# Jonetz/TreeDetection

Hardware: AMD Instinct MI355X
Metric: tiles/sec (1000x1000 RGB+nDSM) predict_tiles model stage (higher is better)
Workload: dtype f32

## Files before the change

treedetection_amd/csrc/api.cpp:

```cpp
#include "common.h"
#include "detect.h"
#include <cstdarg>
#include <cstdio>
#include <cmath>
#include <cstdlib>
#include <cstring>
#include <vector>


namespace {
td_status scratch(void** p, size_t bytes) {
    TD_HIP_CHECK(hipMalloc(p, bytes ? bytes : 16));
    return TD_OK;
}
}

extern "C" {

void td_model_desc_default(td_model_desc* d) {
    d->num_classes = 1;
    d->precision = TD_PRECISION_FP32;
    d->pre_nms_topk = 1000;
    d->post_nms_topk = 1000;
    d->detections_per_image = 100;
// ... 136 lines not shown
    const char* tenv = getenv("TD_WINO_TILE");
    const bool f43 = head_w || (tenv && atoi(tenv) == 4);
    const int P = f43 ? 36 : 16;
    const size_t T = f43 ? (size_t)B * ((H + 3) / 4) * ((W + 3) / 4) : (size_t)B * ((H + 1) / 2) * ((W + 1) / 2);
    std::vector<float> wh((size_t)Cout * 9 * Cin), uh((size_t)P * Cout * Cin);
    TD_HIP_CHECK(hipMemcpy(wh.data(), w, wh.size() * sizeof(float), hipMemcpyDeviceToHost));
    if (f43) wino43_filter_transform(wh.data(), Cout, Cin, uh.data());
    else wino_filter_transform(wh.data(), Cout, Cin, uh.data());
    void *U = nullptr, *V = nullptr, *Mb = nullptr;
    td_status st;
    if ((st = scratch(&U, uh.size() * 4)) < 0 || (st = scratch(&V, P * T * Cin * 4)) < 0 || (st = scratch(&Mb, P * T * Cout * 4)) < 0) {
        (void)hipFree(U); (void)hipFree(V); (void)hipFree(Mb);
        return st;
    }
    TD_HIP_CHECK(hipMemcpy(U, uh.data(), uh.size() * 4, hipMemcpyHostToDevice));
    const char* folde = getenv("TD_WINO_FOLD");
    const bool fold = f43 && !head_w && folde && atoi(folde) != 0;
    if (fold) TD_REQUIRE(wino43_fused_ok(B, H, W, Cin, Cout), "td_conv2d_winograd_nhwc: TD_WINO_FOLD needs Cin %% 128 == 0, Cout %% 64 == 0");
    const char* fenv = getenv("TD_WINO_FUSED");
    WinoRun r{};
    r.form = fold ? CONV_WINO43_FOLD : f43 ? CONV_WINO43 : CONV_WINO22;
    r.fused_input = !fenv || atoi(fenv) != 0;
    r.slab_tiles = (int)T; r.fold_group = B;
    r.x = x; r.U = static_cast<float*>(U); r.scale = scale; r.bias = bias; r.y = y;
    r.B = B; r.H = H; r.W = W; r.cin = Cin; r.cout = Cout; r.relu = relu;
    r.V = static_cast<float*>(V); r.M = static_cast<float*>(Mb); r.m_mul = 1; r.gemm_cfg = -1;
    r.head_w = head_w; r.head_b = head_b; r.head_y = head_y; r.head_n = head_n;
    st = wino_run(r, s);
    hipError_t herr = hipStreamSynchronize(s);
    (void)hipFree(U); (void)hipFree(V); (void)hipFree(Mb);
    if (st < 0) return st;
    TD_HIP_CHECK(herr);
    return TD_OK;
}

td_status td_resize_tile_u8(const uint8_t* src, int h, int w, int c, uint8_t* dst, int out_h, int out_w,
                            int dst_pitch_px, void* tmp_dev, void* stream) {
    return resize_tile_u8_launch(src, h, w, c, dst, out_h, out_w, dst_pitch_px, tmp_dev, static_cast<hipStream_t>(stream));
}

td_status td_resize_batch_u8(const uint8_t* const* src_tiles, int n, int h, int w, int c, uint8_t* dst, int out_h,
                             int out_w, int dst_pitch_px, int64_t dst_image_stride_bytes, void* tmp_dev, void* stream) {
    return resize_batch_u8_launch(src_tiles, n, h, w, c, dst, out_h, out_w, dst_pitch_px, (size_t)dst_image_stride_bytes,
                                  tmp_dev, static_cast<hipStream_t>(stream));
}
// ... 161 lines not shown
```

treedetection_amd/csrc/common.h:

```cpp
#pragma once
#include <hip/hip_runtime.h>
#include <hip/hip_fp16.h>
#include <cstdint>
#include <cstddef>
#include "../../include/treedet.h"
#include "conv_path.h"
#include <string>
#include <vector>

void td_set_error(const char* fmt, ...);

int td_polygons_json_text(const int32_t* mask_region, const int64_t* mask_offset, const uint32_t* mask_bits, int64_t mask_words,
                          const float* scores, const int32_t* classes, int n, const double* transform, const char* image_id,
                          std::string& out, const char* who);

#define TD_HIP_CHECK(expr)                                                                         \
    do {                                                                                           \
        hipError_t _e = (expr);                                                                    \
        if (_e != hipSuccess) {                                                                    \
            td_set_error("%s failed: %s (%s:%d)", #expr, hipGetErrorString(_e), __FILE__, __LINE__); \
            return TD_ERR_HIP;                                                                     \
        }                                                                                          \
    } while (0)

// ... 99 lines not shown
    {TILE_SPLIT,   1, TILE_F32, false, false, 22, 0,   0,  0},
    {TILE_SPLIT,   2, TILE_F32, false, false, 23, 0,   0,  0},
    {TILE_SPLIT,   3, TILE_F32, false, false, 24, 0,   0,  0},
};
static inline const ConvTile* conv_tile(int id) { return id >= 0 && id < (int)(sizeof TD_CONV_TILES / sizeof *TD_CONV_TILES) ? &TD_CONV_TILES[id] : nullptr; }
static inline bool conv_head_capable(int id, int precision) { return precision == TD_PRECISION_FP16 && conv_tile(id) && conv_tile(id)->head; }
const char* conv_tile_refusal(int id, const ConvArgs& a, int precision);
td_status conv2d_launch(const ConvArgs& a, int precision, hipStream_t stream);
td_status conv_pp8_grouped_launch(ConvArgs a, hipStream_t stream);
void conv_bd_pack(const void* w_ohwi, int elem_bytes, int cout, int kh, int kw, int cin, std::vector<unsigned char>& out);
bool conv_bd_ok(const ConvArgs& a, int precision);
td_status conv_bd_launch(const ConvArgs& a, int precision, int variant, hipStream_t stream);
bool conv_bs_ok(const ConvArgs& a, int precision);
td_status conv_bs_launch(const ConvArgs& a, int precision, hipStream_t stream);
void conv_split_pack(const float* w, int cout, int cin, std::vector<unsigned char>& out, int taps = 1);
bool conv_split_ok(const ConvArgs& a, int precision);
td_status conv_split_launch(const ConvArgs& a, int variant, hipStream_t stream);
td_status wino_gemm_launch(const ConvArgs& a, hipStream_t stream);

struct TailArgs {
    const void* x;
    const void* w2;
    const float* scale2;
    const float* bias2;
    const void* w3;
    const float* scale3;
    const float* bias3;
    const void* res;
    void* y;
    int B, H, W, MID, COUT, M;
// ... 11 lines not shown
void wino_filter_transform(const float* w_ohwi, int N, int C, float* U);
td_status wino43_input_launch(const float* x, int B, int H, int W, int C, float* V, const int* m_dyn, hipStream_t s);
td_status wino43_fused_launch(const float* V, const float* U, int B, int H, int W, int C, int N, const float* scale, const float* bias,
                              int relu, float* y, const int* m_dyn, hipStream_t s);
td_status wino43_output_launch(const float* Mb, int B, int H, int W, int N, const float* scale, const float* bias, int relu,
                               float* y, const int* m_dyn, hipStream_t s);
td_status wino43_output_head_launch(const float* Mb, int B, int H, int W, int N, const float* scale, const float* bias, int relu,
                                    const float* head_w, const float* head_b, float* head_y, int head_n, hipStream_t s);
void wino43_filter_transform(const float* w_ohwi, int N, int C, float* U);
struct WinoRun {
    int form;
    bool fused_input;
    int slab_tiles;
    int fold_group;
    const float *x, *U, *scale, *bias;
    float* y;
    int B, H, W, cin, cout, relu;
    float *V, *M;
    const int* m_dyn;
    int m_mul;
    int gemm_cfg;
    const float *head_w, *head_b;
    float* head_y;
    int head_n;
};
ConvArgs wino_plane_args(const WinoRun& r, int n, long long t0);
ConvArgs wino43_plane_args(const WinoRun& r);
enum { WINO_STEP_INPUT, WINO_STEP_GEMM, WINO_STEP_OUTPUT };
struct WinoHook {
    void* ctx;
// ... 26 lines not shown
```

treedetection_amd/csrc/conv_igemm.hip:

```cpp
#include "common.h"
#include <cstdlib>
#include <type_traits>

#include "conv_tiles.h"

namespace {

template <typename T, typename TO, int MT, int NT, int NSTAGE, int WM, int WN>
__global__ __launch_bounds__(64 * WM * WN, NSTAGE == 1 && MT * NT <= 4 ? 4 : 1)
void conv_igemm_kernel(const ConvArgs a_in) {
    ConvArgs a = a_in;
    if (a.batch_count > 1) {
        const long long bz = blockIdx.y;
        a.x = static_cast<const T*>(a.x) + bz * a.x_bs;
        a.w = static_cast<const T*>(a.w) + bz * a.w_bs;
        a.y = static_cast<TO*>(a.y) + bz * a.y_bs;
    }
    constexpr int THREADS = 64 * WM * WN;
    constexpr int BM = 32 * MT * WM, BN = 32 * NT * WN;
    constexpr int LDROWS = THREADS / 8;
    constexpr int AROWS = BM / LDROWS, BROWS = BN / LDROWS;
    static_assert(BM % LDROWS == 0 && BN % LDROWS == 0 && LDROWS % 16 == 0, "tile / thread-count mismatch");
    constexpr int ES = sizeof(T);
    constexpr int KE = Elem<T>::PER_CHUNK;
// ... 913 lines not shown
    const ConvTile* t = conv_tile(id);
    if (!t) return id < 0 ? nullptr : "no such tile id";
    if (t->family == TILE_RETIRED)
        return "a retired experiment (stream-K / the 4-wave 256x256 tile) that lost to the block tiles and left the library";
    const unsigned prec_bit = precision == TD_PRECISION_FP16 ? TILE_F16 : precision == TD_PRECISION_FP32 ? TILE_F32 : 0;
    if (!(t->prec & prec_bit)) return t->prec == TILE_F16 ? "fp16-only tile" : "fp32-only tile";
    if (t->family == TILE_PP8 && (a.out_mode != 0 || a.batch_count > 1)) return "plain output, no batched launch only";
    if (t->family == TILE_PLANE && !(a.KH == 1 && a.KW == 1 && a.stride == 1 && a.pad == 0 && a.out_mode == 0 && a.res_shift == 0 && !a.out_f32 &&
                                     a.m_off == 0 && a.Cin >= 32 && a.Cin % 32 == 0 && a.M > 0 && a.Cout > 0 && (a.batch_count <= 1 || !a.res) &&
                                     (size_t)a.M * a.Cin * 4 < 0xfffffff0ull - (1u << 20)))
        return "plane-only tile (fp32 1x1, stride 1, no padding, no upsampled residual, Cin a multiple of 32)";
    if (t->family == TILE_BS && !conv_bs_ok(a, precision))
        return "conv_bs_ok failed (1x1, stride 1, 1 / 2 / 4 k-chunks, 128 <= Cout <= 2048, Cout % 8 == 0, packed filters)";
    if (t->family == TILE_BD && !conv_bd_ok(a, precision)) return "conv_bd_ok failed (packed filters, plain output)";
    if (t->family == TILE_SPLIT && !conv_split_ok(a, precision))
        return "conv_split_ok failed (fp32 1x1 without padding, plain output, Cin a multiple of 32, split filter bank)";
    return nullptr;
}

td_status conv2d_launch(const ConvArgs& a, int precision, hipStream_t stream) {
    TD_REQUIRE(precision == TD_PRECISION_FP32 || precision == TD_PRECISION_FP16, "conv2d: bad precision %d", precision);
    int cfg = a.tile_cfg;
    if (cfg < 0) {
        const char* forced = getenv("TD_CONV_CFG");
        if (forced) cfg = atoi(forced);
    }
    if (const char* why = conv_tile_refusal(cfg, a, precision)) {
        if (a.tile_strict || !conv_tile(cfg) || conv_tile(cfg)->family == TILE_RETIRED) {
            td_set_error("conv2d: tile_cfg %d cannot run this launch%s: %s", cfg, a.tile_strict ? " (strict tile selection)" : "", why);
            return TD_ERR_INVALID;
        }
        cfg = -1;
    }
    const int ke = precision == TD_PRECISION_FP16 ? 64 : 32;
    TD_REQUIRE(a.Cin % ke == 0, "conv2d: Cin=%d must be a multiple of %d", a.Cin, ke);
    TD_REQUIRE(a.M > 0 && a.Cout > 0, "conv2d: empty problem (M=%d, Cout=%d)", a.M, a.Cout);
    const size_t es = precision == TD_PRECISION_FP16 ? 2 : 4;
    TD_REQUIRE((size_t)a.B * a.H * a.W * (size_t)a.Cin * es < 0xfffffff0ull - (1u << 20), "conv2d: input tensor must stay below 4 GB (32-bit buffer offsets)");
    TD_REQUIRE((size_t)a.Cout * a.KH * a.KW * a.Cin * es < 0xfffffff0ull - (1u << 20), "conv2d: weight tensor must stay below 4 GB");
    TD_REQUIRE(a.KH * a.KW <= 32, "conv2d: at most 32 filter taps (got %dx%d)", a.KH, a.KW);
    TD_REQUIRE(a.out_mode == 0 || (a.Cout % 32 == 0 && !a.res), "conv2d: bad deconv configuration");
    TD_REQUIRE(!a.head_w || (conv_head_capable(cfg, precision) && a.Cout == 256 && !a.res && a.out_mode == 0 && a.head_y && a.head_n >= 1 && a.head_n <= 32),
               "conv2d: a fused head needs a 256-channel fp16 layer on a tile that owns all its channels (tile id %d)", cfg);
    if (cfg < 0) {
        const bool small_m = a.M <= 64 * 256;
        cfg = a.Cout <= 64 ? (small_m ? 3 : 1) : (small_m ? 2 : 0);
    }
    const ConvTile& t = *conv_tile(cfg);
    if (t.family == TILE_BS) return conv_bs_launch(a, precision, stream);
    if (t.family == TILE_BD) return conv_bd_launch(a, precision, t.variant, stream);
    if (t.family == TILE_SPLIT) return conv_split_launch(a, t.variant, stream);
    TD_REQUIRE(a.batch_count <= 1 || (a.KH == 1 && a.KW == 1 && !a.res), "conv2d: batched launches are 1x1 contractions");
    if (t.family == TILE_PP8) return a.out_f32 ? pp8_launch<float>(a, stream) : pp8_launch<_Float16>(a, stream);
    if (t.family == TILE_PLANE) return plane_launch(a, cfg, stream);
    if (precision == TD_PRECISION_FP32) return dispatch<float, float>(a, cfg, stream);
    if (a.out_f32) return dispatch<_Float16, float>(a, cfg, stream);
    return dispatch<_Float16, _Float16>(a, cfg, stream);
}
// ... 1 lines not shown
```

treedetection_amd/csrc/conv_path.cpp:

```cpp
#include "conv_path.h"
#include "../../include/treedet.h"

#include <algorithm>

bool wino43_fused_ok(int B, int H, int W, int C, int N) {
    const long long T = (long long)B * ((H + 3) / 4) * ((W + 3) / 4);
    return (C == 128 || C == 256 || C == 512) && N >= 64 && N % 64 == 0 && 36ull * (unsigned long long)T * C * 4 < 0xfffffff0ull - (1u << 20) &&
           36ull * (unsigned long long)N * C * 4 < 0xfffffff0ull - (1u << 20) && (unsigned long long)B * H * W * N * 4 < 0xfffffff0ull - (1u << 20);
}

ConvPath conv_path(const ConvRules& r, const ConvSite& s) {
    const ConvLayerFacts& L = s.L;
    const int Ho = (s.H + 2 * s.pad - L.kh) / s.stride + 1, Wo = (s.W + 2 * s.pad - L.kw) / s.stride + 1;
    const bool fp32 = r.precision == TD_PRECISION_FP32;
    const int maxc = std::max(L.cin, L.cout);
    ConvPath p{};
    p.head = HEAD_OWN_LAUNCH;
    p.slab_tiles = r.wino_slab > 0 ? r.wino_slab : (1 << 30);
    auto key = [&](int k2, long long rows, int flags) {
        p.tune = true;
        p.key[0] = L.cout; p.key[1] = L.cin; p.key[2] = k2; p.key[3] = (int)rows; p.key[4] = flags;
    };
    const bool head1x1 = s.has_head && r.fuse_head && !s.m_dyn && s.relu && L.cout == 256 && s.head.cin == 256 && s.head.kh == 1 && s.head.kw == 1 &&
                         s.head.cout <= 32 && !s.head.scale;
// ... 19 lines not shown
    }
    const int hw = s.H * s.W, wf = r.wino_fold;
    const bool head = s.has_head, dyn = s.m_dyn;
    const bool fold = wf > 0 && wino43_fused_ok(dyn ? s.B : 1, s.H, s.W, L.cin, L.cout) &&
                      (((wf & 1) && !dyn && (!head || (wf & 32)) && ((L.cin == 256 && hw >= 160 * 160) || (L.cin == 128 && hw >= 80 * 80))) ||
                       ((wf & 2) && dyn && !head) || ((wf & 4) && !dyn && !head && L.cin == 256 && hw >= 80 * 80) ||
                       ((wf & 8) && !dyn && !head && hw >= 40 * 40) || ((wf & 16) && !dyn && !head));
    if (fold) {
        p.form = CONV_WINO43_FOLD;
        const unsigned long long room = 0xfffffff0ull - (2u << 20);
        const unsigned long long gmax = std::min(room / (36ull * tiles_img * (unsigned long long)maxc * 4ull), room / (16ull * tiles_img * L.cout * 4ull));
        p.fold_group = dyn ? s.B : (int)std::max<unsigned long long>(1ull, std::min<unsigned long long>(gmax, s.B));
        return p;
    }
    p.form = CONV_WINO43;
    key(1 * 16 + 1, T43, 4 + 64);
    if (head1x1) p.head = HEAD_IN_TRANSFORM;
    return p;
}
```

treedetection_amd/csrc/conv_path.h:

```cpp
#pragma once
#include <cstddef>

struct ConvRules {
    int precision;
    bool winograd;
    bool wino_fused;
    int wino_minc;
    int wino43_min;
    int wino_fold;
    int wino_slab;
    bool fuse_head;
    size_t wino_elems;
};
struct ConvLayerFacts {
    int cout, cin, kh, kw;
    bool scale, out_f32;
    bool wino_u, wino_u43, w_split;
};
struct ConvSite {
    ConvLayerFacts L;
    int B, H, W, stride, pad;
    bool relu, res;
    int out_mode;
    bool m_dyn;
    int m_mul;
    bool has_head;
    ConvLayerFacts head;
};

enum ConvForm { CONV_DIRECT, CONV_SPLIT, CONV_WINO22, CONV_WINO43, CONV_WINO43_FOLD };
enum ConvHead { HEAD_OWN_LAUNCH, HEAD_IN_TRANSFORM, HEAD_IF_TILE_OWNS_256 };

struct ConvPath {
    ConvForm form;
    ConvHead head;
    bool tune;
    int key[5];
    int slab_tiles;
    int fold_group;
};

ConvPath conv_path(const ConvRules& r, const ConvSite& s);

bool wino43_fused_ok(int B, int H, int W, int C, int N);
```

treedetection_amd/csrc/conv_split.hip:

```cpp
#include "common.h"
#include "conv_tiles.h"
#include <utility>

namespace {

typedef unsigned u32x4 __attribute__((ext_vector_type(4)));

template <int... R, class F>
__device__ __forceinline__ void static_for(std::integer_sequence<int, R...>, F&& f) {
    (f(std::integral_constant<int, R>{}), ...);
}

template <int MT, int NT, int WM, int WN>
__device__ __forceinline__ void conv_split_body(const ConvArgs& a, char* lds) {
    constexpr int THREADS = 64 * WM * WN;
    constexpr int BM = 32 * MT * WM, BN = 32 * NT * WN;
    constexpr int LDROWS = THREADS / 8;
    constexpr int AROWS = BM / LDROWS;
    static_assert(BM % LDROWS == 0 && AROWS >= 1 && LDROWS % 16 == 0, "tile / thread-count mismatch");
    char* As = lds;

    int M = a.M;
    if (a.m_dyn) {
        int md = *a.m_dyn * a.m_mul - a.m_off;
// ... 188 lines not shown
            step(std::integral_constant<int, 1>{}, std::integral_constant<int, 1>{}, it + 1);
        }
        if (it + 2 < nit) {
            step(std::integral_constant<int, 2>{}, std::integral_constant<int, 0>{}, it + 2);
            step(std::integral_constant<int, 2>{}, std::integral_constant<int, 1>{}, it + 2);
        }
    }
    asm volatile("s_waitcnt vmcnt(0)" ::: "memory");
    asm volatile("s_waitcnt lgkmcnt(0)" ::: "memory");
    __builtin_amdgcn_s_barrier();
    conv_epilogue<float, float, MT, NT, WM, WN, 1>(a, acc, lds, M, m0, n0, tid, lane, wm, wn);
}

template <int MT, int NT, int WM, int WN, int WPE>
__global__ __launch_bounds__(64 * WM * WN, WPE)
void conv_split_kernel(const ConvArgs a) {
    constexpr int STAGE_BYTES = 3 * 32 * MT * WM * CHUNK_BYTES;
    constexpr int EPI_BYTES = conv_epilogue_lds_bytes<float, MT, NT, WM, WN, 1>();
    constexpr int LDS_BYTES = STAGE_BYTES > EPI_BYTES ? STAGE_BYTES : EPI_BYTES;
    constexpr int BLOCKS_PER_CU = 4 * WPE / (WM * WN) > 0 ? 4 * WPE / (WM * WN) : 1;
    static_assert(LDS_BYTES * BLOCKS_PER_CU <= 160 * 1024, "the blocks the registers allow on a CU must fit its LDS");
    __shared__ __attribute__((aligned(16))) char lds[LDS_BYTES];
    conv_split_body<MT, NT, WM, WN>(a, lds);
}

template <int MT, int NT, int WM, int WN, int WPE>
td_status launch_split(const ConvArgs& a, hipStream_t stream) {
    const int tiles = td_cdiv(a.M, 32 * MT * WM) * td_cdiv(a.Cout, 32 * NT * WN);
    hipLaunchKernelGGL((conv_split_kernel<MT, NT, WM, WN, WPE>), dim3(tiles), dim3(64 * WM * WN), 0, stream, a);
    TD_KERNEL_CHECK();
    return TD_OK;
}

inline unsigned short bf16_rne(float f) {
    unsigned u = __builtin_bit_cast(unsigned, f);
    if ((u & 0x7fffffffu) > 0x7f800000u) return (unsigned short)((u >> 16) | 0x40);
    u += 0x7fffu + ((u >> 16) & 1u);
    return (unsigned short)(u >> 16);
}

}

void conv_split_pack(const float* w, int cout, int cin, std::vector<unsigned char>& out, int taps) {
    const int nit = taps * (cin / 32), nt32 = (cout + 31) / 32;
// ... 5 lines not shown
                for (int l = 0; l < 64; ++l) {
                    const int n = t * 32 + (l & 31), h = l >> 5;
                    if (n >= cout) continue;
                    const int cc = c / taps, tap = c - cc * taps;
                    for (int e = 0; e < 8; ++e) {
                        float v = w[((size_t)n * taps + tap) * cin + (size_t)cc * 32 + 16 * s + 8 * (e >> 2) + 4 * h + (e & 3)];
                        for (int p = 0; p < 3; ++p) {
                            const unsigned short b = bf16_rne(v);
                            o[(((((size_t)t * nit + c) * 2 + s) * 3 + p) * 64 + l) * 8 + e] = b;
                            v = v - __builtin_bit_cast(float, (unsigned)b << 16);
                        }
                    }
                }
}

bool conv_split_ok(const ConvArgs& a, int precision) {
    return precision == TD_PRECISION_FP32 && a.w_split && a.KH == 1 && a.KW == 1 && a.pad == 0 && a.stride >= 1 && a.out_mode == 0 &&
           a.batch_count <= 1 && !a.out_f32 && !a.head_w && a.Cin >= 32 && a.Cin % 32 == 0 &&
           (size_t)((a.Cout + 31) / 32) * (size_t)(a.Cin / 32) * SPLIT_CHUNK_BYTES < 0xfffffff0ull - (1u << 20);
}

td_status conv_split_launch(const ConvArgs& a, int variant, hipStream_t stream) {
    TD_REQUIRE(conv_split_ok(a, TD_PRECISION_FP32), "split-bf16 contraction: unsupported launch (fp32 1x1 without padding, split filter bank)");
    switch (variant) {
        case 3: return launch_split<2, 2, 1, 2, 2>(a, stream);
        case 2: return launch_split<2, 4, 1, 2, 1>(a, stream);
        case 1: return launch_split<2, 2, 2, 2, 2>(a, stream);
        default: return launch_split<4, 2, 1, 4, 1>(a, stream);
    }
}
```

treedetection_amd/csrc/engine.cpp:

```cpp
#include "common.h"
#include "detect.h"
#include "workspace.h"

#include <cmath>
#include <cstdio>
#include <cstdlib>
#include <cstring>
#include <algorithm>
#include <functional>
#include <map>
#include <optional>
#include <string>
#include <tuple>
#include <vector>

namespace {

struct HostTensor {
    const float* data = nullptr;
    std::vector<int64_t> shape;
    int64_t numel() const {
        int64_t n = 1;
        for (auto s : shape) n *= s;
        return n;
    }
};

enum { SPLIT_FC = 1, SPLIT_LATERAL = 2, SPLIT_CONV1 = 4, SPLIT_CONV3 = 8, SPLIT_SHORTCUT = 16,
       SPLIT_DEFAULT = SPLIT_FC | SPLIT_LATERAL | SPLIT_CONV1 | SPLIT_SHORTCUT };

struct ConvLayer {
    int cout = 0, cin = 0, kh = 1, kw = 1;
    void* w = nullptr;
    float* scale = nullptr;
    float* bias = nullptr;
    bool out_f32 = false;
    void* w_frag = nullptr;
    void* w_split = nullptr;
    void* w_tail_split = nullptr;
    float* wino_u = nullptr;
    float* wino_u43 = nullptr;
};

struct Block {
    ConvLayer c1, c2, c3, sc;
    bool has_sc = false;
    int stride = 1;
};

struct NamedTensor { void* p; WsDims dims; int elem; };

}

struct td_engine : Workspace {
    td_model_desc desc{};
    int device = 0;
// ... 22 lines not shown
    int backbone_subbatch = 0;
    std::map<std::tuple<int, int, int, int, int>, int> tuned;
    bool winograd = true;
    size_t wino_elems = 0;
    bool group_levels = true;
    bool fuse_head = true;
    bool fuse_tail = true;
    bool fuse_tail_fp16 = false;
    bool wino_fused = true;
    int wino_slab = 0;
    int wino_minc = 128;
    int wino43_min = 12;
    int wino_fold = 39;
    int f32_split = SPLIT_DEFAULT;
    bool f32_split_tail = true;
    std::string tune_cache;
    void* tune_evict = nullptr;
    size_t tune_evict_bytes = 0;

    struct FwdCtx {
        const void* images = nullptr;
        int input_format = 0, B = 0, Hp = 0, Wp = 0;
        ImgSizes valid{}, outsz{};
        td_detections out{};
        bool valid_ctx = false;
    } ctx;
    hipEvent_t phase_ev[7] = {};
    bool phase_ev_recorded[7] = {};
    hipEvent_t prev5_ev = nullptr;
    bool prev5_recorded = false;
// ... 136 lines not shown
        td_set_error("load_weights: norm tensors of '%s' do not have %d channels", p.c_str(), c);
        return TD_ERR_WEIGHTS;
    }
    scale.resize(c);
    bias.resize(c);
    for (int i = 0; i < c; ++i) {
        const float r = 1.0f / std::sqrt(v->data[i] + 1e-5f);
        const float s = g->data[i] * r;
        const float ms = m->data[i] * s;
        scale[i] = s;
        bias[i] = b->data[i] - ms;
    }
    return TD_OK;
}

td_status upload_wino(td_engine* e, const std::vector<float>& w_ohwi, ConvLayer& L) {
    L.wino_u = nullptr;
    if (e->desc.precision != TD_PRECISION_FP32 || !e->winograd || L.kh != 3 || L.kw != 3 || L.cin % 32 != 0 || L.cout % 4 != 0)
        return TD_OK;
    std::vector<float> u((size_t)16 * L.cout * L.cin);
    wino_filter_transform(w_ohwi.data(), L.cout, L.cin, u.data());
    td_status st = upload(e, u, &L.wino_u);
    if (st < 0 || e->wino43_min <= 0 || L.cin < e->wino_minc || L.cout < e->wino_minc) return st;
    std::vector<float> u43((size_t)36 * L.cout * L.cin);
    wino43_filter_transform(w_ohwi.data(), L.cout, L.cin, u43.data());
    return upload(e, u43, &L.wino_u43);
}

td_status load_conv_bn(td_engine* e, const TensorMap& tm, const std::string& p, ConvLayer& L, int split_cls = 0) {
    const HostTensor* w;
    td_status st = need(tm, p + ".weight", 4, &w);
    if (st < 0) return st;
    L.cout = (int)w->shape[0];
    L.cin = (int)w->shape[1];
    L.kh = (int)w->shape[2];
    L.kw = (int)w->shape[3];
    const std::vector<float> packed = pack_ohwi(*w);
    if ((st = upload_w(e, packed, &L.w)) < 0) return st;
    if ((st = upload_frag(e, packed, L)) < 0) return st;
    if ((st = upload_split(e, packed, L, split_cls)) < 0) return st;
    if ((st = upload_wino(e, packed, L)) < 0) return st;
    std::vector<float> s, b;
    if ((st = bn_fold(tm, p, L.cout, s, b)) < 0) return st;
    if ((st = upload(e, s, &L.scale)) < 0) return st;
    return upload(e, b, &L.bias);
}

td_status load_conv_bias(td_engine* e, const TensorMap& tm, const std::string& p, ConvLayer& L, int split_cls = 0) {
    const HostTensor *w, *b;
    td_status st = need(tm, p + ".weight", 4, &w);
    if (st < 0) return st;
    if ((st = need(tm, p + ".bias", 1, &b)) < 0) return st;
    L.cout = (int)w->shape[0];
    L.cin = (int)w->shape[1];
    L.kh = (int)w->shape[2];
    L.kw = (int)w->shape[3];
    if (b->shape[0] != L.cout) {
        td_set_error("load_weights: bias of '%s' has wrong length", p.c_str());
        return TD_ERR_WEIGHTS;
    }
    const std::vector<float> packed = pack_ohwi(*w);
    if ((st = upload_w(e, packed, &L.w)) < 0) return st;
    if ((st = upload_frag(e, packed, L)) < 0) return st;
    if ((st = upload_split(e, packed, L, split_cls)) < 0) return st;
    if ((st = upload_wino(e, packed, L)) < 0) return st;
    L.scale = nullptr;
    return upload(e, std::vector<float>(b->data, b->data + L.cout), &L.bias);
}

WsGeom engine_geom(const td_engine* e, int B, int Hp, int Wp) {
    int32_t c[WS_WIDTHS] = {e->stem_c};
    for (int s = 0; s < 4; ++s) { c[1 + s] = e->stages[s][0].c1.cout; c[5 + s] = e->stages[s][0].c2.cout; c[9 + s] = e->stages[s][0].c3.cout; }
    c[13] = e->fpn_c; c[14] = e->fc_dim; c[15] = e->deconv.cout / 4;
    return ws_geom(e->desc.precision, e->winograd, e->desc.post_nms_topk, e->desc.detections_per_image, c, B, Hp, Wp);
}

void publish(td_engine* e, const WsGeom& g, int phase) {
    for (const WsRow& r : ws_rows())
        for (int i = 0; r.pub && (r.phase == phase || (phase == 0 && r.phase == TD_PHASE_STEM)) && i < r.count; ++i) {
            char name[32];
// ... 107 lines not shown
    TD_REQUIRE(d.precision == TD_PRECISION_FP32 || d.precision == TD_PRECISION_FP16, "td_engine_create: bad precision %d", d.precision);
    TD_REQUIRE(d.pre_nms_topk >= 1 && d.pre_nms_topk <= RPN_CAND, "td_engine_create: pre_nms_topk must be in [1,%d]", RPN_CAND);
    TD_REQUIRE(d.post_nms_topk >= 1 && d.post_nms_topk <= 1024, "td_engine_create: post_nms_topk must be in [1,1024]");
    TD_REQUIRE(d.detections_per_image >= 1 && d.detections_per_image <= 1024, "td_engine_create: detections_per_image must be in [1,1024]");
    int ndev = 0;
    TD_HIP_CHECK(hipGetDeviceCount(&ndev));
    TD_REQUIRE(device >= 0 && device < ndev, "td_engine_create: device %d of %d", device, ndev);
    TD_HIP_CHECK(hipSetDevice(device));
    td_engine* e = new td_engine();
    if (const char* sbenv = getenv("TD_BACKBONE_SUBBATCH")) e->backbone_subbatch = atoi(sbenv);
    if (const char* tc = getenv("TD_TUNE_CACHE")) e->tune_cache = tc;
    if (const char* gl = getenv("TD_GROUP_LEVELS")) e->group_levels = atoi(gl) != 0;
    if (const char* ft = getenv("TD_FUSE_TAIL")) { e->fuse_tail = atoi(ft) != 0; e->fuse_tail_fp16 = atoi(ft) == 2; }
    if (const char* sp = getenv("TD_F32_SPLIT")) e->f32_split = atoi(sp);
    if (const char* spt = getenv("TD_F32_SPLIT_TAIL")) e->f32_split_tail = atoi(spt) != 0;
    e->desc = d;
    read_rule_switches(e);
    load_tune_cache(e);
    e->device = device;
    *out = e;
    return TD_OK;
}

void td_engine_destroy(td_engine* e) {
    if (!e) return;
    (void)hipSetDevice(e->device);
    free_pool(e->weight_allocs);
    free_pool(e->ws_allocs);
    if (e->tune_evict) (void)hipFree(e->tune_evict);
    for (auto& r : e->prof_recs) { (void)hipEventDestroy(r.a); (void)hipEventDestroy(r.b); }
// ... 68 lines not shown
            std::vector<unsigned short> w16;
            std::vector<float> b16;
            stem_mfma_prepare(p.data(), s.data(), b.data(), e->stem_c, w16, b16);
            if ((st = upload(e, w16, &e->stem_w16)) < 0) return st;
            if ((st = upload(e, b16, &e->stem_bias16)) < 0) return st;
        }
    }
    for (int si = 0; si < 4; ++si) {
        e->stages[si].clear();
        for (int bi = 0;; ++bi) {
            const std::string p = "backbone.bottom_up.res" + std::to_string(si + 2) + "." + std::to_string(bi);
            if (tm.find(p + ".conv1.weight") == tm.end()) break;
            Block blk;
            blk.stride = (bi == 0 && si > 0) ? 2 : 1;
            if ((st = load_conv_bn(e, tm, p + ".conv1", blk.c1, si > 0 ? SPLIT_CONV1 : 0)) < 0) return st;
            if ((st = load_conv_bn(e, tm, p + ".conv2", blk.c2)) < 0) return st;
            if ((st = load_conv_bn(e, tm, p + ".conv3", blk.c3, si > 0 ? SPLIT_CONV3 : 0)) < 0) return st;
            if (si == 0 && (st = upload_tail_split(e, pack_ohwi(tm.at(p + ".conv2.weight")), blk.c2, blk.c3.cout)) < 0) return st;
            blk.has_sc = tm.find(p + ".shortcut.weight") != tm.end();
            if (blk.has_sc && (st = load_conv_bn(e, tm, p + ".shortcut", blk.sc, si > 0 ? SPLIT_SHORTCUT : 0)) < 0) return st;
            e->stages[si].push_back(blk);
        }
        if (e->stages[si].empty()) {
            td_set_error("load_weights: no blocks found for res%d", si + 2);
            return TD_ERR_WEIGHTS;
        }
    }
    for (int l = 0; l < 4; ++l) {
        if ((st = load_conv_bias(e, tm, "backbone.fpn_lateral" + std::to_string(l + 2), e->lateral[l], SPLIT_LATERAL)) < 0) return st;
        if ((st = load_conv_bias(e, tm, "backbone.fpn_output" + std::to_string(l + 2), e->fpn_out[l])) < 0) return st;
    }
    e->fpn_c = e->lateral[0].cout;
    if ((st = load_conv_bias(e, tm, "proposal_generator.rpn_head.conv", e->rpn_conv)) < 0) return st;
    {
        const HostTensor *wo, *bo, *wd, *bd;
        if ((st = need(tm, "proposal_generator.rpn_head.objectness_logits.weight", 4, &wo)) < 0) return st;
        if ((st = need(tm, "proposal_generator.rpn_head.objectness_logits.bias", 1, &bo)) < 0) return st;
        if ((st = need(tm, "proposal_generator.rpn_head.anchor_deltas.weight", 4, &wd)) < 0) return st;
        if ((st = need(tm, "proposal_generator.rpn_head.anchor_deltas.bias", 1, &bd)) < 0) return st;
        if (wo->shape[0] != RPN_A || wd->shape[0] != 4 * RPN_A || wo->shape[1] != e->fpn_c || wd->shape[1] != e->fpn_c) {
            td_set_error("load_weights: RPN head must have %d anchors per position", RPN_A);
            return TD_ERR_WEIGHTS;
        }
        const int c = e->fpn_c;
        std::vector<float> w((size_t)RPN_HEAD_C * c), b(RPN_HEAD_C);
        std::memcpy(w.data(), wo->data, sizeof(float) * RPN_A * c);
        std::memcpy(w.data() + (size_t)RPN_A * c, wd->data, sizeof(float) * 4 * RPN_A * c);
        std::memcpy(b.data(), bo->data, sizeof(float) * RPN_A);
// ... 207 lines not shown
    hipStream_t s;
    const WinoRun& r;
    std::optional<ClassScope> cs;
    static void begin(void* ctx, int step, long long n) {
        WinoBooks& k = *static_cast<WinoBooks*>(ctx);
        const WinoRun& r = k.r;
        if (r.m_dyn) {
            k.cs.emplace(k.e, k.s, TD_CLS_MASK_HEAD, 0.0, 0.0);
            return;
        }
        const bool f22 = r.form == CONV_WINO22;
        const double P = f22 ? 16.0 : 36.0;
        const double T = f22 ? (double)n : (double)r.B * ((r.H + 3) / 4) * ((r.W + 3) / 4);
        const double share = f22 ? 1.0 : (double)n / r.B;
        const double px = (double)r.B * r.H * r.W;
        const double xb = 4.0 * px * r.cin, yb = 4.0 * px * r.cout, ub = 4.0 * P * r.cout * r.cin;
        const double vb = 4.0 * P * T * r.cin, mb = 4.0 * P * T * r.cout, pf = 2.0 * P * T * (double)r.cin * r.cout;
        if (step == WINO_STEP_INPUT) {
            k.cs.emplace(k.e, k.s, TD_CLS_WINO_XFORM, 0.0, (xb + vb) * share);
        } else if (step == WINO_STEP_GEMM) {
            k.cs.emplace(k.e, k.s, TD_CLS_WINO_GEMM, pf * share,
                         r.form == CONV_WINO43_FOLD ? (vb + yb) * share + ub : (f22 && r.fused_input ? xb : vb) + ub + mb);
        } else if (r.head_w) {
            k.cs.emplace(k.e, k.s, TD_CLS_WINO_XFORM, 2.0 * px * r.head_n * r.cout, mb + (4.0 * px * r.head_n + 4.0 * r.head_n * r.cout));
        } else {
            k.cs.emplace(k.e, k.s, TD_CLS_WINO_XFORM, 0.0, mb + yb);
        }
    }
    static void end(void* ctx) { static_cast<WinoBooks*>(ctx)->cs.reset(); }
};

td_status run_wino(td_engine* e, const WinoRun& r, hipStream_t s) {
    if (!e->prof) return wino_run(r, s);
    WinoBooks books{e, s, r, std::nullopt};
    const WinoHook hook{&books, WinoBooks::begin, WinoBooks::end};
    return wino_run(r, s, &hook);
}

ConvLayerFacts layer_facts(const ConvLayer& L) {
    return {L.cout, L.cin, L.kh, L.kw, L.scale != nullptr, L.out_f32, L.wino_u != nullptr, L.wino_u43 != nullptr, L.w_split != nullptr};
}

td_status run_conv(td_engine* e, const ConvLayer& L, const void* x_, int B_, int H_, int W_, int stride, int pad, bool relu, void* y_,
                   const void* res_, int res_shift, hipStream_t s_, const int* m_dyn = nullptr, int m_mul = 1, int out_mode = 0,
                   const ConvLayer* head = nullptr, float* head_y = nullptr, bool* head_fused = nullptr) {
    const int prec_ = e->desc.precision;
    const ConvSite site{layer_facts(L), B_, H_, W_, stride, pad, relu, res_ != nullptr, out_mode, m_dyn != nullptr, m_mul,
                        head != nullptr, head ? layer_facts(*head) : ConvLayerFacts{}};
    const ConvPath path = conv_path(conv_rules(e), site);
    const bool split = path.form == CONV_SPLIT, use_wino = path.form >= CONV_WINO22, use_43 = path.form >= CONV_WINO43;
    const int Ho = (H_ + 2 * pad - L.kh) / stride + 1, Wo = (W_ + 2 * pad - L.kw) / stride + 1;
    const double M = (double)B_ * Ho * Wo, K = (double)L.kh * L.kw * L.cin;
    const double flops = 2.0 * M * L.cout * K;
    const double es = prec_ == TD_PRECISION_FP16 ? 2.0 : 4.0;
    const double bytes = es * ((double)B_ * H_ * W_ * L.cin / (stride * stride) + M * L.cout * (res_ ? 2.0 : 1.0)) + (split ? 6.0 : es) * L.cout * K;
    td_status st2;
    ConvArgs ca{};
    ca.x = x_; ca.w = L.w; ca.w_frag = L.w_frag; ca.w_split = split ? L.w_split : nullptr; ca.scale = L.scale; ca.bias = L.bias; ca.res = res_; ca.y = y_;
    ca.B = B_; ca.H = H_; ca.W = W_; ca.Cin = L.cin; ca.Cout = L.cout; ca.KH = L.kh; ca.KW = L.kw;
    ca.stride = stride; ca.pad = pad; ca.Ho = Ho; ca.Wo = Wo;
    ca.res_shift = res_shift; ca.relu = relu ? 1 : 0; ca.out_mode = out_mode;
    ca.M = B_ * Ho * Wo; ca.m_dyn = m_dyn; ca.m_mul = m_mul; ca.tile_cfg = -1; ca.out_f32 = L.out_f32 ? 1 : 0;
    WinoRun wr{};
    if (use_wino) {
        wr.form = path.form; wr.fused_input = e->wino_fused; wr.slab_tiles = path.slab_tiles; wr.fold_group = path.fold_group;
        wr.x = static_cast<const float*>(x_); wr.U = use_43 ? L.wino_u43 : L.wino_u; wr.scale = L.scale; wr.bias = L.bias; wr.y = static_cast<float*>(y_);
        wr.B = B_; wr.H = H_; wr.W = W_; wr.cin = L.cin; wr.cout = L.cout; wr.relu = relu ? 1 : 0;
        wr.V = e->wino_v; wr.M = e->wino_m; wr.m_dyn = m_dyn; wr.m_mul = m_mul; wr.gemm_cfg = -1;
    }
    if (path.tune) {
        const auto key = std::make_tuple(path.key[0], path.key[1], path.key[2], path.key[3], path.key[4]);
        if (use_wino) {
            auto wino = [&](int c) { WinoRun q = wr; q.gemm_cfg = c; return run_wino(e, q, s_); };
            st2 = tuned_cfg(e, key, prec_, use_43 ? wino43_plane_args(wr) : wino_plane_args(wr, path.key[3], 0), s_, wino, &wr.gemm_cfg);
        } else {
            auto direct = [&](int c) { ConvArgs a = ca; a.tile_cfg = c; return conv2d_launch(a, prec_, s_); };
            st2 = tuned_cfg(e, key, prec_, ca, s_, direct, &ca.tile_cfg);
        }
        if (st2 < 0) return st2;
    }
    const bool fuse_head = path.head == HEAD_IN_TRANSFORM || (path.head == HEAD_IF_TILE_OWNS_256 && conv_head_capable(ca.tile_cfg, prec_));
    if (head_fused) *head_fused = fuse_head;
    const double hflops = fuse_head ? 2.0 * M * head->cout * L.cout : 0.0, hbytes = fuse_head ? 4.0 * M * head->cout + es * head->cout * L.cout : 0.0;
    ProfScope ps(e, s_, m_dyn ? 7 : 0, m_dyn ? 0.0 : flops, m_dyn ? 0.0 : bytes);
    if (e->prof && !m_dyn) {
        const double padded = use_43 ? (double)(((H_ + 3) / 4) * 4) * (((W_ + 3) / 4) * 4) / ((double)H_ * W_) : 1.0;
        e->prof_flops[8] += use_43 ? flops * padded * 0.25 : (use_wino ? flops * 4.0 / 9.0 : (split ? flops * 6.0 / 16.0 : flops));
        e->prof_launches[8] += use_wino ? 1 : 0;
    }
    if (e->prof && fuse_head) {
        e->prof_flops[0] += hflops;
        e->prof_flops[8] += hflops;
        e->prof_launches[0] += 1;
        e->prof_bytes[0] += hbytes + es * M * L.cout;
    }
    if (use_wino) {
        if (fuse_head) { wr.head_w = static_cast<const float*>(head->w); wr.head_b = head->bias; wr.head_y = head_y; wr.head_n = head->cout; }
        return run_wino(e, wr, s_);
    }
    const int cls = m_dyn ? TD_CLS_MASK_HEAD : (H_ == 1 && W_ == 1 ? TD_CLS_FC : (L.kh == 1 && L.kw == 1 ? TD_CLS_CONV1X1 : TD_CLS_CONV3X3));
    if (fuse_head) {
        ca.head_w = head->w; ca.head_b = head->bias; ca.head_y = head_y; ca.head_n = head->cout;
// ... 464 lines not shown
```

treedetection_amd/csrc/wino_seq.cpp:

```cpp
#include "common.h"

#include <algorithm>

ConvArgs wino_plane_args(const WinoRun& r, int n, long long t0) {
    ConvArgs a{};
    a.w = r.U; a.y = r.M;
    a.Cin = r.cin; a.Cout = r.cout; a.KH = a.KW = 1; a.stride = 1; a.pad = 0;
    a.M = n; a.m_dyn = r.m_dyn; a.m_mul = r.m_dyn ? r.m_mul / 4 : 1;
    a.m_off = (int)t0;
    a.w_bs = (long long)r.cout * r.cin; a.y_bs = (long long)n * r.cout;
    a.tile_cfg = r.gemm_cfg;
    if (r.fused_input) { a.x = r.x; a.B = r.B; a.H = r.H; a.W = r.W; }
    else { a.x = r.V; a.B = 1; a.H = 1; a.W = n; a.Ho = 1; a.Wo = n; a.batch_count = 16; a.x_bs = (long long)n * r.cin; }
    return a;
}

ConvArgs wino43_plane_args(const WinoRun& r) {
    const int tiles_img = ((r.H + 3) / 4) * ((r.W + 3) / 4);
    const long long T = (long long)r.B * tiles_img;
    ConvArgs a{};
    a.x = r.V; a.w = r.U; a.y = r.M;
    a.Cin = r.cin; a.Cout = r.cout; a.KH = a.KW = 1; a.stride = 1; a.pad = 0;
    a.B = 1; a.H = 1; a.W = (int)T; a.Ho = 1; a.Wo = (int)T;
    a.M = (int)T; a.m_dyn = r.m_dyn; a.m_mul = r.m_dyn ? tiles_img : 1;
    a.batch_count = 36; a.x_bs = T * r.cin; a.w_bs = (long long)r.cout * r.cin; a.y_bs = T * r.cout;
    a.tile_cfg = r.gemm_cfg;
    return a;
}

td_status wino_run(const WinoRun& r, hipStream_t s, const WinoHook* hook) {
#define TD_WINO_STEP(which, n, launch)                  \
    do {                                                \
        if (hook) hook->begin(hook->ctx, which, n);     \
        const td_status st_ = (launch);                 \
        if (hook) hook->end(hook->ctx);                 \
        if (st_ < 0) return st_;                        \
    } while (0)
    if (r.form == CONV_WINO22) {
        const long long T = (long long)r.B * ((r.H + 1) / 2) * ((r.W + 1) / 2);
        for (long long t0 = 0; t0 < T; t0 += r.slab_tiles) {
            const int n = (int)std::min<long long>(r.slab_tiles, T - t0);
// ... 25 lines not shown
```

Baseline: 747.5.

## Run Winograd F(4,3) batched plane GEMMs on split-bf16 filter banks

Packs the 36 Winograd F(4,3) transformed filter planes into split-bf16 banks at load time and routes the batched plane GEMM to the split-bf16 tile kernels, which gain a blockIdx.y batch dimension. This is enabled by default for res stages 2+, the FPN output convs and the RPN conv. It replaces the fp32 GEMM with emulated-fp32 split-precision matrix math to use the faster matrix units, at the cost of extra filter memory and a small accuracy risk.

```diff
diff --git a/treedetection_amd/csrc/api.cpp b/treedetection_amd/csrc/api.cpp
--- a/treedetection_amd/csrc/api.cpp
+++ b/treedetection_amd/csrc/api.cpp
@@ -174,6 +174,18 @@
         return st;
     }
     TD_HIP_CHECK(hipMemcpy(U, uh.data(), uh.size() * 4, hipMemcpyHostToDevice));
+    const char* spe = getenv("TD_WINO_SPLIT");
+    void* Us = nullptr;
+    auto free_all = [&]() { (void)hipFree(U); (void)hipFree(V); (void)hipFree(Mb); (void)hipFree(Us); };
+    if (f43 && spe && atoi(spe) != 0) {
+        std::vector<unsigned char> packed;
+        conv_split_pack_planes(uh.data(), 36, Cout, Cin, packed);
+        if ((st = scratch(&Us, packed.size())) < 0 || hipMemcpy(Us, packed.data(), packed.size(), hipMemcpyHostToDevice) != hipSuccess) {
+            free_all();
+            if (st < 0) return st;
+            TD_REQUIRE(false, "td_conv2d_winograd_nhwc: copying the split twin of the filter bank failed");
+        }
+    }
     const char* folde = getenv("TD_WINO_FOLD");
     const bool fold = f43 && !head_w && folde && atoi(folde) != 0;
     if (fold) TD_REQUIRE(wino43_fused_ok(B, H, W, Cin, Cout), "td_conv2d_winograd_nhwc: TD_WINO_FOLD needs Cin %% 128 == 0, Cout %% 64 == 0");
@@ -182,13 +194,13 @@
     r.form = fold ? CONV_WINO43_FOLD : f43 ? CONV_WINO43 : CONV_WINO22;
     r.fused_input = !fenv || atoi(fenv) != 0;
     r.slab_tiles = (int)T; r.fold_group = B;
-    r.x = x; r.U = static_cast<float*>(U); r.scale = scale; r.bias = bias; r.y = y;
+    r.x = x; r.U = static_cast<float*>(U); r.U_split = Us; r.scale = scale; r.bias = bias; r.y = y;
     r.B = B; r.H = H; r.W = W; r.cin = Cin; r.cout = Cout; r.relu = relu;
     r.V = static_cast<float*>(V); r.M = static_cast<float*>(Mb); r.m_mul = 1; r.gemm_cfg = -1;
     r.head_w = head_w; r.head_b = head_b; r.head_y = head_y; r.head_n = head_n;
     st = wino_run(r, s);
     hipError_t herr = hipStreamSynchronize(s);
-    (void)hipFree(U); (void)hipFree(V); (void)hipFree(Mb);
+    free_all();
     if (st < 0) return st;
     TD_HIP_CHECK(herr);
     return TD_OK;
diff --git a/treedetection_amd/csrc/common.h b/treedetection_amd/csrc/common.h
--- a/treedetection_amd/csrc/common.h
+++ b/treedetection_amd/csrc/common.h
@@ -137,6 +137,8 @@
 bool conv_bs_ok(const ConvArgs& a, int precision);
 td_status conv_bs_launch(const ConvArgs& a, int precision, hipStream_t stream);
 void conv_split_pack(const float* w, int cout, int cin, std::vector<unsigned char>& out, int taps = 1);
+size_t conv_split_bank_bytes(int cout, int cin);
+void conv_split_pack_planes(const float* u, int planes, int cout, int cin, std::vector<unsigned char>& out);
 bool conv_split_ok(const ConvArgs& a, int precision);
 td_status conv_split_launch(const ConvArgs& a, int variant, hipStream_t stream);
 td_status wino_gemm_launch(const ConvArgs& a, hipStream_t stream);
@@ -178,6 +180,7 @@
     int slab_tiles;
     int fold_group;
     const float *x, *U, *scale, *bias;
+    const void* U_split;
     float* y;
     int B, H, W, cin, cout, relu;
     float *V, *M;
diff --git a/treedetection_amd/csrc/conv_igemm.hip b/treedetection_amd/csrc/conv_igemm.hip
--- a/treedetection_amd/csrc/conv_igemm.hip
+++ b/treedetection_amd/csrc/conv_igemm.hip
@@ -951,7 +951,8 @@
         return "conv_bs_ok failed (1x1, stride 1, 1 / 2 / 4 k-chunks, 128 <= Cout <= 2048, Cout % 8 == 0, packed filters)";
     if (t->family == TILE_BD && !conv_bd_ok(a, precision)) return "conv_bd_ok failed (packed filters, plain output)";
     if (t->family == TILE_SPLIT && !conv_split_ok(a, precision))
-        return "conv_split_ok failed (fp32 1x1 without padding, plain output, Cin a multiple of 32, split filter bank)";
+        return "conv_split_ok failed (fp32 1x1 without padding, plain output, Cin a multiple of 32, split filter bank; batched: plain planes with static rows)";
+    if (t->family != TILE_SPLIT && a.w_split && a.batch_count > 1) return "batched split planes run the split-bf16 tiles only";
     return nullptr;
 }
 
@@ -979,6 +980,10 @@
     TD_REQUIRE(a.out_mode == 0 || (a.Cout % 32 == 0 && !a.res), "conv2d: bad deconv configuration");
     TD_REQUIRE(!a.head_w || (conv_head_capable(cfg, precision) && a.Cout == 256 && !a.res && a.out_mode == 0 && a.head_y && a.head_n >= 1 && a.head_n <= 32),
                "conv2d: a fused head needs a 256-channel fp16 layer on a tile that owns all its channels (tile id %d)", cfg);
+    if (cfg < 0 && a.w_split && a.batch_count > 1) {
+        TD_REQUIRE(conv_split_ok(a, precision), "conv2d: batched split planes need plain fp32 planes with static rows and the split bank's byte stride");
+        cfg = a.M <= 2048 ? 37 : 35;
+    }
     if (cfg < 0) {
         const bool small_m = a.M <= 64 * 256;
         cfg = a.Cout <= 64 ? (small_m ? 3 : 1) : (small_m ? 2 : 0);
diff --git a/treedetection_amd/csrc/conv_path.cpp b/treedetection_amd/csrc/conv_path.cpp
--- a/treedetection_amd/csrc/conv_path.cpp
+++ b/treedetection_amd/csrc/conv_path.cpp
@@ -57,7 +57,8 @@
         return p;
     }
     p.form = CONV_WINO43;
-    key(1 * 16 + 1, T43, 4 + 64);
+    p.split_planes = L.w_split && !dyn;
+    key(1 * 16 + 1, T43, 4 + 64 + (p.split_planes ? 128 : 0));
     if (head1x1) p.head = HEAD_IN_TRANSFORM;
     return p;
 }
diff --git a/treedetection_amd/csrc/conv_path.h b/treedetection_amd/csrc/conv_path.h
--- a/treedetection_amd/csrc/conv_path.h
+++ b/treedetection_amd/csrc/conv_path.h
@@ -38,6 +38,7 @@
     int key[5];
     int slab_tiles;
     int fold_group;
+    bool split_planes;
 };
 
 ConvPath conv_path(const ConvRules& r, const ConvSite& s);
diff --git a/treedetection_amd/csrc/conv_split.hip b/treedetection_amd/csrc/conv_split.hip
--- a/treedetection_amd/csrc/conv_split.hip
+++ b/treedetection_amd/csrc/conv_split.hip
@@ -1,6 +1,8 @@
 #include "common.h"
 #include "conv_tiles.h"
+#include <algorithm>
 #include <utility>
+#include <vector>
 
 namespace {
 
@@ -226,7 +228,14 @@
 
 template <int MT, int NT, int WM, int WN, int WPE>
 __global__ __launch_bounds__(64 * WM * WN, WPE)
-void conv_split_kernel(const ConvArgs a) {
+void conv_split_kernel(const ConvArgs a_in) {
+    ConvArgs a = a_in;
+    if (a.batch_count > 1) {
+        const long long bz = blockIdx.y;
+        a.x = static_cast<const float*>(a.x) + bz * a.x_bs;
+        a.w_split = static_cast<const char*>(a.w_split) + bz * a.w_bs;
+        a.y = static_cast<float*>(a.y) + bz * a.y_bs;
+    }
     constexpr int STAGE_BYTES = 3 * 32 * MT * WM * CHUNK_BYTES;
     constexpr int EPI_BYTES = conv_epilogue_lds_bytes<float, MT, NT, WM, WN, 1>();
     constexpr int LDS_BYTES = STAGE_BYTES > EPI_BYTES ? STAGE_BYTES : EPI_BYTES;
@@ -239,7 +248,7 @@
 template <int MT, int NT, int WM, int WN, int WPE>
 td_status launch_split(const ConvArgs& a, hipStream_t stream) {
     const int tiles = td_cdiv(a.M, 32 * MT * WM) * td_cdiv(a.Cout, 32 * NT * WN);
-    hipLaunchKernelGGL((conv_split_kernel<MT, NT, WM, WN, WPE>), dim3(tiles), dim3(64 * WM * WN), 0, stream, a);
+    hipLaunchKernelGGL((conv_split_kernel<MT, NT, WM, WN, WPE>), dim3(tiles, a.batch_count > 1 ? a.batch_count : 1), dim3(64 * WM * WN), 0, stream, a);
     TD_KERNEL_CHECK();
     return TD_OK;
 }
@@ -275,10 +284,24 @@
                 }
 }
 
+size_t conv_split_bank_bytes(int cout, int cin) { return (size_t)((cout + 31) / 32) * (size_t)(cin / 32) * SPLIT_CHUNK_BYTES; }
+
+void conv_split_pack_planes(const float* u, int planes, int cout, int cin, std::vector<unsigned char>& out) {
+    const size_t bank = conv_split_bank_bytes(cout, cin);
+    out.resize((size_t)planes * bank);
+    std::vector<unsigned char> one;
+    for (int p = 0; p < planes; ++p) {
+        conv_split_pack(u + (size_t)p * cout * cin, cout, cin, one);
+        std::copy(one.begin(), one.end(), out.begin() + (size_t)p * bank);
+    }
+}
+
 bool conv_split_ok(const ConvArgs& a, int precision) {
+    const size_t bank = (size_t)((a.Cout + 31) / 32) * (size_t)(a.Cin / 32) * SPLIT_CHUNK_BYTES;
+    const bool planes_ok = a.batch_count <= 1 || (!a.res && !a.m_dyn && a.m_off == 0 && a.stride == 1 && (long long)a.B * a.H * a.W == a.M &&
+                                                  a.x_bs >= (long long)a.M * a.Cin && a.y_bs >= (long long)a.M * a.Cout && a.w_bs == (long long)bank);
     return precision == TD_PRECISION_FP32 && a.w_split && a.KH == 1 && a.KW == 1 && a.pad == 0 && a.stride >= 1 && a.out_mode == 0 &&
-           a.batch_count <= 1 && !a.out_f32 && !a.head_w && a.Cin >= 32 && a.Cin % 32 == 0 &&
-           (size_t)((a.Cout + 31) / 32) * (size_t)(a.Cin / 32) * SPLIT_CHUNK_BYTES < 0xfffffff0ull - (1u << 20);
+           planes_ok && !a.out_f32 && !a.head_w && a.Cin >= 32 && a.Cin % 32 == 0 && bank < 0xfffffff0ull - (1u << 20);
 }
 
 td_status conv_split_launch(const ConvArgs& a, int variant, hipStream_t stream) {
diff --git a/treedetection_amd/csrc/engine.cpp b/treedetection_amd/csrc/engine.cpp
--- a/treedetection_amd/csrc/engine.cpp
+++ b/treedetection_amd/csrc/engine.cpp
@@ -28,6 +28,7 @@
 
 enum { SPLIT_FC = 1, SPLIT_LATERAL = 2, SPLIT_CONV1 = 4, SPLIT_CONV3 = 8, SPLIT_SHORTCUT = 16,
        SPLIT_DEFAULT = SPLIT_FC | SPLIT_LATERAL | SPLIT_CONV1 | SPLIT_SHORTCUT };
+enum { WINO_SPLIT_RES = 1, WINO_SPLIT_FPN = 2, WINO_SPLIT_RPN = 4, WINO_SPLIT_DEFAULT = WINO_SPLIT_RES | WINO_SPLIT_FPN | WINO_SPLIT_RPN };
 
 struct ConvLayer {
     int cout = 0, cin = 0, kh = 1, kw = 1;
@@ -40,6 +41,7 @@
     void* w_tail_split = nullptr;
     float* wino_u = nullptr;
     float* wino_u43 = nullptr;
+    void* wino_u43_split = nullptr;
 };
 
 struct Block {
@@ -92,6 +94,7 @@
     int wino_fold = 39;
     int f32_split = SPLIT_DEFAULT;
     bool f32_split_tail = true;
+    int f32_split_wino = WINO_SPLIT_DEFAULT;
     std::string tune_cache;
     void* tune_evict = nullptr;
     size_t tune_evict_bytes = 0;
@@ -258,8 +261,9 @@
     return TD_OK;
 }
 
-td_status upload_wino(td_engine* e, const std::vector<float>& w_ohwi, ConvLayer& L) {
+td_status upload_wino(td_engine* e, const std::vector<float>& w_ohwi, ConvLayer& L, int wino_cls) {
     L.wino_u = nullptr;
+    L.wino_u43_split = nullptr;
     if (e->desc.precision != TD_PRECISION_FP32 || !e->winograd || L.kh != 3 || L.kw != 3 || L.cin % 32 != 0 || L.cout % 4 != 0)
         return TD_OK;
     std::vector<float> u((size_t)16 * L.cout * L.cin);
@@ -268,10 +272,16 @@
     if (st < 0 || e->wino43_min <= 0 || L.cin < e->wino_minc || L.cout < e->wino_minc) return st;
     std::vector<float> u43((size_t)36 * L.cout * L.cin);
     wino43_filter_transform(w_ohwi.data(), L.cout, L.cin, u43.data());
-    return upload(e, u43, &L.wino_u43);
-}
-
-td_status load_conv_bn(td_engine* e, const TensorMap& tm, const std::string& p, ConvLayer& L, int split_cls = 0) {
+    if ((st = upload(e, u43, &L.wino_u43)) < 0 || !(e->f32_split_wino & wino_cls)) return st;
+    std::vector<unsigned char> packed;
+    conv_split_pack_planes(u43.data(), 36, L.cout, L.cin, packed);
+    unsigned char* d = nullptr;
+    st = upload(e, packed, &d);
+    L.wino_u43_split = d;
+    return st;
+}
+
+td_status load_conv_bn(td_engine* e, const TensorMap& tm, const std::string& p, ConvLayer& L, int split_cls = 0, int wino_cls = 0) {
     const HostTensor* w;
     td_status st = need(tm, p + ".weight", 4, &w);
     if (st < 0) return st;
@@ -283,14 +293,14 @@
     if ((st = upload_w(e, packed, &L.w)) < 0) return st;
     if ((st = upload_frag(e, packed, L)) < 0) return st;
     if ((st = upload_split(e, packed, L, split_cls)) < 0) return st;
-    if ((st = upload_wino(e, packed, L)) < 0) return st;
+    if ((st = upload_wino(e, packed, L, wino_cls)) < 0) return st;
     std::vector<float> s, b;
     if ((st = bn_fold(tm, p, L.cout, s, b)) < 0) return st;
     if ((st = upload(e, s, &L.scale)) < 0) return st;
     return upload(e, b, &L.bias);
 }
 
-td_status load_conv_bias(td_engine* e, const TensorMap& tm, const std::string& p, ConvLayer& L, int split_cls = 0) {
+td_status load_conv_bias(td_engine* e, const TensorMap& tm, const std::string& p, ConvLayer& L, int split_cls = 0, int wino_cls = 0) {
     const HostTensor *w, *b;
     td_status st = need(tm, p + ".weight", 4, &w);
     if (st < 0) return st;
@@ -307,7 +317,7 @@
     if ((st = upload_w(e, packed, &L.w)) < 0) return st;
     if ((st = upload_frag(e, packed, L)) < 0) return st;
     if ((st = upload_split(e, packed, L, split_cls)) < 0) return st;
-    if ((st = upload_wino(e, packed, L)) < 0) return st;
+    if ((st = upload_wino(e, packed, L, wino_cls)) < 0) return st;
     L.scale = nullptr;
     return upload(e, std::vector<float>(b->data, b->data + L.cout), &L.bias);
 }
@@ -445,6 +455,7 @@
     if (const char* ft = getenv("TD_FUSE_TAIL")) { e->fuse_tail = atoi(ft) != 0; e->fuse_tail_fp16 = atoi(ft) == 2; }
     if (const char* sp = getenv("TD_F32_SPLIT")) e->f32_split = atoi(sp);
     if (const char* spt = getenv("TD_F32_SPLIT_TAIL")) e->f32_split_tail = atoi(spt) != 0;
+    if (const char* spw = getenv("TD_F32_SPLIT_WINO")) e->f32_split_wino = atoi(spw);
     e->desc = d;
     read_rule_switches(e);
     load_tune_cache(e);
@@ -543,7 +554,7 @@
             Block blk;
             blk.stride = (bi == 0 && si > 0) ? 2 : 1;
             if ((st = load_conv_bn(e, tm, p + ".conv1", blk.c1, si > 0 ? SPLIT_CONV1 : 0)) < 0) return st;
-            if ((st = load_conv_bn(e, tm, p + ".conv2", blk.c2)) < 0) return st;
+            if ((st = load_conv_bn(e, tm, p + ".conv2", blk.c2, 0, si >= 2 ? WINO_SPLIT_RES : 0)) < 0) return st;
             if ((st = load_conv_bn(e, tm, p + ".conv3", blk.c3, si > 0 ? SPLIT_CONV3 : 0)) < 0) return st;
             if (si == 0 && (st = upload_tail_split(e, pack_ohwi(tm.at(p + ".conv2.weight")), blk.c2, blk.c3.cout)) < 0) return st;
             blk.has_sc = tm.find(p + ".shortcut.weight") != tm.end();
@@ -557,10 +568,10 @@
     }
     for (int l = 0; l < 4; ++l) {
         if ((st = load_conv_bias(e, tm, "backbone.fpn_lateral" + std::to_string(l + 2), e->lateral[l], SPLIT_LATERAL)) < 0) return st;
-        if ((st = load_conv_bias(e, tm, "backbone.fpn_output" + std::to_string(l + 2), e->fpn_out[l])) < 0) return st;
+        if ((st = load_conv_bias(e, tm, "backbone.fpn_output" + std::to_string(l + 2), e->fpn_out[l], 0, WINO_SPLIT_FPN)) < 0) return st;
     }
     e->fpn_c = e->lateral[0].cout;
-    if ((st = load_conv_bias(e, tm, "proposal_generator.rpn_head.conv", e->rpn_conv)) < 0) return st;
+    if ((st = load_conv_bias(e, tm, "proposal_generator.rpn_head.conv", e->rpn_conv, 0, WINO_SPLIT_RPN)) < 0) return st;
     {
         const HostTensor *wo, *bo, *wd, *bd;
         if ((st = need(tm, "proposal_generator.rpn_head.objectness_logits.weight", 4, &wo)) < 0) return st;
@@ -798,8 +809,9 @@
         const double T = f22 ? (double)n : (double)r.B * ((r.H + 3) / 4) * ((r.W + 3) / 4);
         const double share = f22 ? 1.0 : (double)n / r.B;
         const double px = (double)r.B * r.H * r.W;
-        const double xb = 4.0 * px * r.cin, yb = 4.0 * px * r.cout, ub = 4.0 * P * r.cout * r.cin;
-        const double vb = 4.0 * P * T * r.cin, mb = 4.0 * P * T * r.cout, pf = 2.0 * P * T * (double)r.cin * r.cout;
+        const bool splitp = r.form == CONV_WINO43 && r.U_split;
+        const double xb = 4.0 * px * r.cin, yb = 4.0 * px * r.cout, ub = (splitp ? 6.0 : 4.0) * P * r.cout * r.cin;
+        const double vb = 4.0 * P * T * r.cin, mb = 4.0 * P * T * r.cout, pf = 2.0 * P * T * (double)r.cin * r.cout * (splitp ? 6.0 / 16.0 : 1.0);
         if (step == WINO_STEP_INPUT) {
             k.cs.emplace(k.e, k.s, TD_CLS_WINO_XFORM, 0.0, (xb + vb) * share);
         } else if (step == WINO_STEP_GEMM) {
@@ -822,7 +834,7 @@
 }
 
 ConvLayerFacts layer_facts(const ConvLayer& L) {
-    return {L.cout, L.cin, L.kh, L.kw, L.scale != nullptr, L.out_f32, L.wino_u != nullptr, L.wino_u43 != nullptr, L.w_split != nullptr};
+    return {L.cout, L.cin, L.kh, L.kw, L.scale != nullptr, L.out_f32, L.wino_u != nullptr, L.wino_u43 != nullptr, L.w_split != nullptr || L.wino_u43_split != nullptr};
 }
 
 td_status run_conv(td_engine* e, const ConvLayer& L, const void* x_, int B_, int H_, int W_, int stride, int pad, bool relu, void* y_,
@@ -851,6 +863,7 @@
         wr.x = static_cast<const float*>(x_); wr.U = use_43 ? L.wino_u43 : L.wino_u; wr.scale = L.scale; wr.bias = L.bias; wr.y = static_cast<float*>(y_);
         wr.B = B_; wr.H = H_; wr.W = W_; wr.cin = L.cin; wr.cout = L.cout; wr.relu = relu ? 1 : 0;
         wr.V = e->wino_v; wr.M = e->wino_m; wr.m_dyn = m_dyn; wr.m_mul = m_mul; wr.gemm_cfg = -1;
+        wr.U_split = path.split_planes ? L.wino_u43_split : nullptr;
     }
     if (path.tune) {
         const auto key = std::make_tuple(path.key[0], path.key[1], path.key[2], path.key[3], path.key[4]);
@@ -869,7 +882,7 @@
     ProfScope ps(e, s_, m_dyn ? 7 : 0, m_dyn ? 0.0 : flops, m_dyn ? 0.0 : bytes);
     if (e->prof && !m_dyn) {
         const double padded = use_43 ? (double)(((H_ + 3) / 4) * 4) * (((W_ + 3) / 4) * 4) / ((double)H_ * W_) : 1.0;
-        e->prof_flops[8] += use_43 ? flops * padded * 0.25 : (use_wino ? flops * 4.0 / 9.0 : (split ? flops * 6.0 / 16.0 : flops));
+        e->prof_flops[8] += use_43 ? flops * padded * 0.25 * (path.split_planes ? 6.0 / 16.0 : 1.0) : (use_wino ? flops * 4.0 / 9.0 : (split ? flops * 6.0 / 16.0 : flops));
         e->prof_launches[8] += use_wino ? 1 : 0;
     }
     if (e->prof && fuse_head) {
diff --git a/treedetection_amd/csrc/wino_seq.cpp b/treedetection_amd/csrc/wino_seq.cpp
--- a/treedetection_amd/csrc/wino_seq.cpp
+++ b/treedetection_amd/csrc/wino_seq.cpp
@@ -25,6 +25,7 @@
     a.M = (int)T; a.m_dyn = r.m_dyn; a.m_mul = r.m_dyn ? tiles_img : 1;
     a.batch_count = 36; a.x_bs = T * r.cin; a.w_bs = (long long)r.cout * r.cin; a.y_bs = T * r.cout;
     a.tile_cfg = r.gemm_cfg;
+    if (r.U_split && !r.m_dyn) { a.w_split = r.U_split; a.w_bs = (long long)conv_split_bank_bytes(r.cout, r.cin); }
     return a;
 }
 
```

After: 768.7, median of 6. 1.03x the previous value.
